# prakharg24/yoloret

Hardware: AMD Instinct MI355X
Metric: images/sec (+ p50 per-image ms) MobileNetV2-0.75x @416, 1/2/4/8 MI355X (higher is better)
Workload: dtype f32; 1 GPU; mobilenetv2x75 @416, batch 64 per GPU, fp32, random weights (SURVEY 8(d) recipe; parity tests run the variance-preserving recipe, see DESIGN.md 5), C=20: forward + decode + per-class NMS + pack; 3 steps in flight (each step = one whole batch on its own HIP stream and workspace); global_batch=64, parallelism=dp1 (image-sharded)

## Files before the change

### yoloret_amd/csrc/pointwise_stream.hip

```cpp
#include <algorithm>
#include <cstdlib>

#include "pws_common.h"
#include "mbr_common.h"

typedef __attribute__((address_space(3))) void* pwt_lds_ptr;

struct PwtDiv { unsigned m; int s; };
static inline PwtDiv pwt_div_make(unsigned d) {
    if (d <= 1) return {0u, -1};
    int l = 0;
    while ((1u << l) < d) ++l;
    const unsigned long long m = ((1ull << (31 + l)) + d - 1) / d;
    return {(unsigned)m, l - 1};
}
__device__ __forceinline__ int pwt_div(int n, PwtDiv d) { return d.s < 0 ? n : (int)(__umulhi((unsigned)n, d.m) >> d.s); }

struct PwtArgs {
    const float* planes;
    unsigned plane_bytes;
    int T;
    int csplit;
    int nwg;
    int ntiles;
    PwtDiv d_hw, d_wq, d_hwq;
    unsigned in_bytes, out_bytes, gate_bytes;
    int TA, quad;
    unsigned out2_bytes;
};

#ifndef PWT_MAX_WAVES
#define PWT_MAX_WAVES 16
#endif
constexpr int pwt_waves_fit(int nk, int rows, int mode);
constexpr int pwt_waves(int nk, int rows, int mode) { return pwt_waves_fit(nk, rows, mode) < PWT_MAX_WAVES ? pwt_waves_fit(nk, rows, mode) : PWT_MAX_WAVES; }
constexpr int pwt_waves_fit(int nk, int rows, int mode) {
    const int nkr = nk * rows;
    if (mode == 0) return nkr <= 6 ? 16 : nkr <= 10 ? 12 : 8;
    if (mode == 1) return nkr <= 9 ? 16 : nkr <= 12 ? 12 : 8;
    if (rows == 1) return nk <= 8 ? 16 : nk <= 10 ? 12 : 8;
    return nk <= 2 ? 16 : nk <= 4 ? 12 : 8;
}

#ifdef PWT_TIMING
__device__ unsigned pwt_dbg[256 * 16 * 8];
extern "C" int yr_pwt_dbg_read(unsigned* dst, int n) { return (int)hipMemcpyFromSymbol(dst, HIP_SYMBOL(pwt_dbg), (size_t)n * 4); }
#define PWT_T(i) { __builtin_amdgcn_sched_barrier(0); const unsigned long long t_ = __builtin_amdgcn_s_memtime(); tacc[i] += t_ - tlast; tlast = t_; __builtin_amdgcn_sched_barrier(0); }
#else
#define PWT_T(i)
#endif

__device__ __forceinline__ int pwt_pixel_of_row(const PwArgs& a, const PwtArgs& x, int m) {
    if (!x.quad) return m;
    const int q = m >> 2, sub = m & 3;
    const int wq = a.W >> 1, hwq = (a.H >> 1) * wq;
    const int b = pwt_div(q, x.d_hwq), r = q - b * hwq;
    const int yq = pwt_div(r, x.d_wq), xq = r - yq * wq;
    return (b * a.H + 2 * yq + (sub >> 1)) * a.W + 2 * xq + (sub & 1);
}

template <int NK, int ROWS, int MODE>
__global__ __launch_bounds__(64 * pwt_waves(NK, ROWS, MODE)) void pwt_kernel(PwArgs a, PwtArgs x) {
    constexpr int NW = pwt_waves(NK, ROWS, MODE), TB = NK * 2048;
    typedef unsigned u4 __attribute__((ext_vector_type(4)));
    extern __shared__ __attribute__((aligned(16))) char lds_raw[];
    const int lane = threadIdx.x & 63, li = lane & 15, g = lane >> 4;
    const int w = __builtin_amdgcn_readfirstlane(threadIdx.x >> 6);
    const int part = blockIdx.x % x.csplit, wg = blockIdx.x / x.csplit;
    const int t0 = part * x.T / x.csplit, t1 = (part + 1) * x.T / x.csplit, run = t1 - t0;
    float* const ss = reinterpret_cast<float*>(lds_raw + (size_t)run * TB);
#ifdef PWT_TIMING
    unsigned long long tacc[8] = {0, 0, 0, 0, 0, 0, 0, 0}, tlast = __builtin_amdgcn_s_memtime();
#endif

    {
        const yr_rsrc wsrc = yr_make_rsrc(x.planes, x.plane_bytes);
        const int npiece = run * NK * 2;
        for (int p = w; p < npiece; p += NW)
            __builtin_amdgcn_raw_ptr_buffer_load_lds(wsrc, (pwt_lds_ptr)(lds_raw + p * 1024), 16, (unsigned)(t0 * TB + p * 1024 + lane * 16), 0, 0, 0);
    }
    const int bn_i = (int)threadIdx.x;
    const int bn_n = bn_i < 16 * run && (a.out2 != nullptr || 16 * t0 + bn_i < a.N) ? 16 * t0 + bn_i : 0;
    const float bn_sl = (a.scale ? a.scale : x.planes)[bn_n], bn_hl = (a.shift ? a.shift : x.planes)[bn_n];

    const int kp = a.S.kp;
    const int stride = x.nwg * NW;
    int tile = wg + x.nwg * w;
    const yr_rsrc xsrc = yr_make_rsrc(a.S.s[0].ptr, x.in_bytes), osrc = yr_make_rsrc(a.out, x.out_bytes);
    const yr_rsrc osrc2 = yr_make_rsrc(a.out2 ? a.out2 : a.out, a.out2 ? x.out2_bytes : 16u);
    const yr_rsrc gsrc = yr_make_rsrc(MODE == 2 ? a.gate : a.S.s[0].ptr, MODE == 2 ? x.gate_bytes : 16u);
    PwRow<0> row[MODE == 0 ? ROWS : 1];
    float4 xa[ROWS][NK][2];
    int cv[MODE == 0 ? ROWS : 1][MODE == 0 ? NK : 1][2];
    unsigned goff[ROWS];
    int pix[ROWS];
    constexpr int GQ = 2, NGQ = (NK + GQ - 1) / GQ;
    float4 gq[MODE == 2 ? 2 : 1][MODE == 2 ? ROWS : 1][GQ][2];
    auto gate_issue = [&](auto J) __attribute__((always_inline)) {
        constexpr int j = decltype(J)::value;
        if constexpr (MODE == 2 && j < NGQ) {
            pw_unroll<ROWS * GQ * 2>([&](auto U) __attribute__((always_inline)) {
                constexpr int u = decltype(U)::value, i = u / (2 * GQ), cc = (u / 2) % GQ, q = u % 2, c = j * GQ + cc;
                const int k = c * 32 + g * 8 + 4 * q;
                if constexpr (c < NK) gq[j & 1][i][cc][q] = __builtin_bit_cast(float4, __builtin_amdgcn_raw_buffer_load_b128(gsrc, k < kp ? goff[i] + 4u * k : YR_DEAD, 0, 0));
            });
        }
    };
    const int csrc = a.S.s[0].c, ldsrc = a.S.s[0].ld;
    auto fetch = [&]() __attribute__((always_inline)) {
#pragma unroll
        for (int i = 0; i < ROWS; ++i) {
            const int m = (tile * ROWS + i) * 16 + li;
            if constexpr (MODE == 0) {
                row[i].init(a, m);
                pix[i] = pw_pixel_of_row(a, m < a.M ? m : 0);
                pw_unroll<NK * 2>([&](auto U) __attribute__((always_inline)) {
                    constexpr int u = decltype(U)::value, c = u / 2, q = u % 2;
                    float4 unused;
                    row[i].template issue<false>(a, c * 32 + g * 8 + 4 * q, kp, xa[i][c][q], unused, cv[i][c][q]);
                });
            } else {
                const int mm = pwt_pixel_of_row(a, x, m < a.M ? m : 0);
                pix[i] = mm;
                const unsigned poff = (unsigned)mm * (unsigned)ldsrc * 4u;
                if constexpr (MODE == 2) goff[i] = (unsigned)pwt_div(mm, x.d_hw) * (unsigned)a.gate_ld * 4u;
                pw_unroll<NK * 2>([&](auto U) __attribute__((always_inline)) {
                    constexpr int u = decltype(U)::value, c = u / 2, q = u % 2;
                    const int k = c * 32 + g * 8 + 4 * q;
                    xa[i][c][q] = __builtin_bit_cast(float4, __builtin_amdgcn_raw_buffer_load_b128(xsrc, (m < a.M && k < kp) ? poff + 4u * k : YR_DEAD, 0, 0));
                });
            }
        }
        gate_issue(std::integral_constant<int, 0>{});
    };
    auto no_fetch = [&]() __attribute__((always_inline)) {
        pw_unroll<ROWS * NK * 2>([&](auto U) __attribute__((always_inline)) {
            constexpr int u = decltype(U)::value;
            xa[u / (2 * NK)][(u / 2) % NK][u % 2] = make_float4(0.f, 0.f, 0.f, 0.f);
            if constexpr (MODE == 0) cv[u / (2 * NK)][(u / 2) % NK][u % 2] = 0;
        });
    };
    if (tile < x.ntiles) fetch();
    else no_fetch();
    PWT_T(0)
    if (bn_i < 16 * run) { ss[bn_i] = a.scale ? bn_sl : 1.f; ss[16 * run + bn_i] = a.shift ? bn_hl : 0.f; }
    __builtin_amdgcn_s_waitcnt(0x0070);
    __syncthreads();
    PWT_T(1)

    const f32x4 k11 = {0.00048828125f, 0.00048828125f, 0.00048828125f, 0.00048828125f};
    const bool ragged = (csrc & 3) != 0, clamp = a.act != YR_ACT_NONE;
    while (tile < x.ntiles) {
        pws_u4 xh[ROWS][NK], xm[ROWS][NK];
        pw_unroll<ROWS * NK>([&](auto U) __attribute__((always_inline)) {
            constexpr int u = decltype(U)::value, c = u / ROWS, i = u % ROWS;
            float4 v0 = xa[i][c][0], v1 = xa[i][c][1];
            if constexpr (MODE == 0) {
                v0 = pw_finish<1>(v0, v0, cv[i][c][0]);
                v1 = pw_finish<1>(v1, v1, cv[i][c][1]);
            } else {
                const int k0 = c * 32 + g * 8;
                if constexpr (MODE == 2) {
                    if constexpr (i == 0 && c % GQ == 0) gate_issue(std::integral_constant<int, c / GQ + 1>{});
                    const float4 g0 = gq[(c / GQ) & 1][i][c % GQ][0], g1 = gq[(c / GQ) & 1][i][c % GQ][1];
                    v0 = make_float4(v0.x * g0.x, v0.y * g0.y, v0.z * g0.z, v0.w * g0.w);
                    v1 = make_float4(v1.x * g1.x, v1.y * g1.y, v1.z * g1.z, v1.w * g1.w);
                }
                if (ragged) {
                    v0 = pw_finish<1>(v0, v0, csrc - k0);
                    v1 = pw_finish<1>(v1, v1, csrc - k0 - 4);
                }
            }
            unsigned h[4], mm[4];
            yr_cut2(v0.x, v0.y, h[0], mm[0]);
            yr_cut2(v0.z, v0.w, h[1], mm[1]);
            yr_cut2(v1.x, v1.y, h[2], mm[2]);
            yr_cut2(v1.z, v1.w, h[3], mm[3]);
            xh[i][c] = (pws_u4){h[0], h[1], h[2], h[3]};
            xm[i][c] = (pws_u4){mm[0], mm[1], mm[2], mm[3]};
        });
        PWT_T(2)
        unsigned obase[ROWS], obase2[ROWS];
#pragma unroll
        for (int i = 0; i < ROWS; ++i) {
            const int m = (tile * ROWS + i) * 16 + li;
            const bool keep = m < a.M && (!a.pool || (li & 3) == 0), keep2 = m < a.M && (!a.pool2 || (li & 3) == 0);
            obase[i] = keep ? (unsigned)(a.pool ? m >> 2 : pix[i]) * (unsigned)a.out_ld * 4u : YR_DEAD;
            obase2[i] = keep2 && a.out2 ? (unsigned)(a.pool2 ? m >> 2 : pix[i]) * (unsigned)a.out2_ld * 4u : YR_DEAD;
        }
        for (int t = 0; t < run; ++t) {
            const pws_u4* fe = reinterpret_cast<const pws_u4*>(lds_raw + (size_t)t * TB) + lane;
            f32x4 acc[ROWS], ac1[ROWS];
#pragma unroll
            for (int i = 0; i < ROWS; ++i) { acc[i] = (f32x4){0.f, 0.f, 0.f, 0.f}; ac1[i] = acc[i]; }
#pragma unroll
            for (int c = 0; c < NK; ++c) {
                const pws_u4 wh = fe[(2 * c) * 64], wm = fe[(2 * c + 1) * 64];
#pragma unroll
                for (int i = 0; i < ROWS; ++i) acc[i] = pws_mfma(wh, xh[i][c], acc[i]);
#pragma unroll
                for (int i = 0; i < ROWS; ++i) ac1[i] = pws_mfma(wh, xm[i][c], ac1[i]);
#pragma unroll
                for (int i = 0; i < ROWS; ++i) ac1[i] = pws_mfma(wm, xh[i][c], ac1[i]);
            }
            const f32x4 sc = *reinterpret_cast<const f32x4*>(ss + 16 * t + 4 * g);
            const f32x4 sh = *reinterpret_cast<const f32x4*>(ss + 16 * run + 16 * t + 4 * g);
            const bool second = t0 + t >= x.TA;
            const int n = 16 * (t0 + t - (second ? x.TA : 0)) + 4 * g, cnt = (second ? a.N2 : a.N) - n;
            const bool clamp_t = second ? a.act2 != YR_ACT_NONE : clamp, pool_t = second ? a.pool2 != 0 : a.pool != 0;
#pragma unroll
            for (int i = 0; i < ROWS; ++i) {
                f32x4 v = __builtin_elementwise_fma(ac1[i], k11, acc[i]);
#pragma unroll
                for (int r = 0; r < 4; ++r) v[r] = __builtin_fmaf(v[r], sc[r], sh[r]);
                if (clamp_t) {
#pragma unroll
                    for (int r = 0; r < 4; ++r) v[r] = __builtin_amdgcn_fmed3f(v[r], 0.f, 6.f);
                }
                if (pool_t) {
#pragma unroll
                    for (int r = 0; r < 4; ++r) {
                        v[r] = fmaxf(v[r], __int_as_float(__builtin_amdgcn_update_dpp(0, __float_as_int(v[r]), 0xB1, 0xf, 0xf, false)));
                        v[r] = fmaxf(v[r], __int_as_float(__builtin_amdgcn_update_dpp(0, __float_as_int(v[r]), 0x4E, 0xf, 0xf, false)));
                    }
                }
                const unsigned ob = second ? obase2[i] : obase[i];
                const unsigned off = ob == YR_DEAD || cnt <= 0 ? YR_DEAD : ob + 4u * (unsigned)n;
                if (second) {
                    if (cnt >= 4) __builtin_amdgcn_raw_buffer_store_b128(__builtin_bit_cast(u4, v), osrc2, off, 0, 0);
                    else {
#pragma unroll
                        for (int r = 0; r < 3; ++r) __builtin_amdgcn_raw_buffer_store_b32(__float_as_uint(v[r]), osrc2, r < cnt ? off + 4u * r : YR_DEAD, 0, 0);
                    }
                } else if (cnt >= 4) {
                    __builtin_amdgcn_raw_buffer_store_b128(__builtin_bit_cast(u4, v), osrc, off, 0, 0);
                } else {
#pragma unroll
                    for (int r = 0; r < 3; ++r) __builtin_amdgcn_raw_buffer_store_b32(__float_as_uint(v[r]), osrc, r < cnt ? off + 4u * r : YR_DEAD, 0, 0);
                }
            }
        }
        PWT_T(3)
        tile += stride;
        if (tile < x.ntiles) fetch();
        else no_fetch();
        PWT_T(4)
#ifdef PWT_TIMING
        tacc[5] += 1;
#endif
    }
#ifdef PWT_TIMING
    __builtin_amdgcn_s_waitcnt(0x0070);
    PWT_T(6)
    if (lane < 8 && blockIdx.x < 256) {
        unsigned tv = 0;
#pragma unroll
        for (int i = 0; i < 8; ++i) tv = lane == i ? (unsigned)tacc[i] : tv;
        pwt_dbg[(blockIdx.x * 16 + w) * 8 + lane] = tv;
    }
#endif
}

template <int NK, int ROWS>
static int launch_pwt(const PwArgs& a, PwtArgs& x, hipStream_t s) {
    const int mode = pw_mode_of(a);
    const int NW = pwt_waves(NK, ROWS, mode);
    x.ntiles = (a.M + 16 * ROWS - 1) / (16 * ROWS);
    int cs = 1;
    while ((x.T + cs - 1) / cs * (size_t)(NK * 2048 + 128) > 150 * 1024 && cs < x.T) ++cs;
    x.csplit = cs;
    const int cus = 256 / cs;
    int aw = (x.ntiles + cus - 1) / cus;
    if (aw > NW) aw = NW;
    x.nwg = (x.ntiles + aw - 1) / aw;
    if (x.nwg > cus) x.nwg = cus;
    const size_t lds = (size_t)((x.T + cs - 1) / cs) * (NK * 2048 + 128);
    YR_REQUIRE(lds <= 160 * 1024 && (x.T + cs - 1) / cs <= 32, "pointwise (pixel-stationary form): %d tiles of %d chunks do not fit LDS", x.T, NK);
    const dim3 grid((unsigned)(x.nwg * cs));
#define PWT_GO(MD) YR_LAUNCH((pwt_kernel<NK, ROWS, MD>), grid, dim3(64 * pwt_waves(NK, ROWS, MD)), lds, 160 * 1024, s, ("pwt_kernel<%d,%d,%d>", NK, ROWS, MD), a, x)
    return mode == 0 ? PWT_GO(0) : mode == 1 ? PWT_GO(1) : PWT_GO(2);
#undef PWT_GO
}

extern "C" int yr_pwt_chunks(int kp) {
    static const int sizes[] = {1, 2, 3, 4, 5, 6, 7, 8, 9, 10, 12, 16};
    const int nk = (kp + 31) / 32;
    for (int v : sizes)
        if (v >= nk) return v;
    return 0;
}

static int pwt_launch_images(const PwArgs& a, hipStream_t s) {
    const int nk = yr_pwt_chunks(a.S.kp);
    YR_REQUIRE(nk > 0, "pointwise (pixel-stationary form): a k space of %d channels is beyond 16 chunks", a.S.kp);
    YR_REQUIRE(a.dw_w == nullptr && a.pre == nullptr && a.res == nullptr, "pointwise (pixel-stationary form): no depthwise-folded source, addend or residual");
    YR_REQUIRE(a.act == YR_ACT_NONE || a.act == YR_ACT_RELU6, "pointwise (pixel-stationary form): activation %d (none and ReLU6 only)", a.act);
    YR_REQUIRE(!pw_any_pooled(a.S), "pointwise (pixel-stationary form): no pooled source");
    PwtArgs x;
    x.TA = (a.N + 15) / 16;
    x.planes = a.wt; x.T = x.TA + (a.out2 ? (a.N2 + 15) / 16 : 0);
    x.quad = a.pool || (a.out2 && a.pool2);
    if (a.out2) YR_REQUIRE(pw_mode_of(a) != 0, "pointwise (pixel-stationary form): two outputs need a single identity source");
    if (a.out2) YR_REQUIRE(a.act2 == YR_ACT_NONE || a.act2 == YR_ACT_RELU6, "pointwise (pixel-stationary form): activation %d of the second output", a.act2);
    if (x.quad) YR_REQUIRE(a.H % 2 == 0 && a.W % 2 == 0, "pointwise (pixel-stationary form): a pooled output needs an even map");
    x.plane_bytes = (unsigned)x.T * (unsigned)nk * 2048u;
    x.d_hw = pwt_div_make((unsigned)(a.H * a.W));
    x.d_wq = pwt_div_make((unsigned)(a.W >> 1 > 0 ? a.W >> 1 : 1));
    x.d_hwq = pwt_div_make((unsigned)((a.H >> 1) * (a.W >> 1) > 0 ? (a.H >> 1) * (a.W >> 1) : 1));
    const long long inb = (long long)a.M * a.S.s[0].ld * 4, outb = (long long)(a.pool ? a.M / 4 : a.M) * a.out_ld * 4;
    YR_REQUIRE(inb < (long long)YR_DEAD && outb < (long long)YR_DEAD, "pointwise (pixel-stationary form): a map of %lld bytes is beyond the 32-bit offsets", inb > outb ? inb : outb);
    x.in_bytes = (unsigned)inb; x.out_bytes = (unsigned)outb;
    const long long outb2 = a.out2 ? (long long)(a.pool2 ? a.M / 4 : a.M) * a.out2_ld * 4 : 0;
    YR_REQUIRE(outb2 < (long long)YR_DEAD, "pointwise (pixel-stationary form): a second output of %lld bytes is beyond the 32-bit offsets", outb2);
    x.out2_bytes = (unsigned)outb2;
    x.gate_bytes = a.gate ? (unsigned)((long long)(a.M / (a.H * a.W)) * a.gate_ld * 4) : 0u;
    const char* rows_env = getenv("YR_PWT_ROWS");
    const bool two = rows_env && atoi(rows_env) == 2 && nk <= 6;
#define PWT_CASE(K) if (nk == K) return two ? launch_pwt<K, 2>(a, x, s) : launch_pwt<K, 1>(a, x, s);
#define PWT_CASE1(K) if (nk == K) return launch_pwt<K, 1>(a, x, s);
#ifdef PWT_ONLY
    PWT_CASE(PWT_ONLY)
#else
    PWT_CASE(1) PWT_CASE(2) PWT_CASE(3) PWT_CASE(4) PWT_CASE(5) PWT_CASE(6) PWT_CASE1(7) PWT_CASE1(8) PWT_CASE1(9) PWT_CASE1(10) PWT_CASE1(12) PWT_CASE1(16)
#endif
#undef PWT_CASE
#undef PWT_CASE1
    return YR_ERR_ARG;
}

int yr_pw_launch_stream(const PwArgs& a0, hipStream_t s) {
    const long long hw = (long long)a0.H * a0.W;
    const int B = (int)(a0.M / hw);
    long long per_image = (a0.pool ? hw / 4 : hw) * a0.out_ld * 4;
    if (a0.out2) per_image = std::max(per_image, (a0.pool2 ? hw / 4 : hw) * a0.out2_ld * 4);
    for (int i = 0; i < a0.S.n; ++i) per_image = std::max(per_image, (long long)a0.S.s[i].h * a0.S.s[i].w * a0.S.s[i].ld * 4);
    const char* lim = getenv("YR_PWT_MAX_BYTES");
    const long long fit = (lim && atoll(lim) > 0 ? atoll(lim) : 0x7e000000ll) / (per_image > 0 ? per_image : 1);
    if (fit >= B || (long long)B * hw != a0.M) return pwt_launch_images(a0, s);
    YR_REQUIRE(fit >= 1, "pointwise (pixel-stationary form): one image's map of %lld bytes is beyond the 32-bit offsets", per_image);
    for (int b0 = 0; b0 < B; b0 += (int)fit) {
        PwArgs a = a0;
        const int n = B - b0 < fit ? B - b0 : (int)fit;
        a.M = (int)(n * hw);
        for (int i = 0; i < a.S.n; ++i) a.S.s[i].ptr += (size_t)b0 * a.S.s[i].h * a.S.s[i].w * a.S.s[i].ld;
        if (a.gate) a.gate += (size_t)b0 * a.gate_ld;
        a.out += (size_t)b0 * (a.pool ? hw / 4 : hw) * a.out_ld;
        if (a.out2) a.out2 += (size_t)b0 * (a.pool2 ? hw / 4 : hw) * a.out2_ld;
        const int rc = pwt_launch_images(a, s);
        if (rc) return rc;
    }
    return YR_OK;
}
```

Baseline: 50960 img/s.

## Rework pixel-stationary pointwise geometry: wider channel split, runtime wave count, async BN loads

Launch geometry now comes from a helper that splits output-channel tiles across more workgroups (about one part per six tiles, capped by available wave slots). When the split leaves slack it drops to 8 waves per workgroup, and the workgroup count accounts for several workgroups sharing a CU's LDS. Wave count becomes a runtime parameter, and an env override is added for tuning. BN scale/shift are now loaded straight into LDS with buffer-to-LDS loads instead of through registers. The start-up wait only drains the weight and BN loads rather than the in-flight pixel fetches, using s_barrier instead of __syncthreads. The 16-wave threshold for rows==1 gate mode is also lowered. The wider split means more redundant activation reads, and the partial vmcnt wait relies on exact load-ordering counts.

```diff
diff --git a/yoloret_amd/csrc/pointwise_stream.hip b/yoloret_amd/csrc/pointwise_stream.hip
--- a/yoloret_amd/csrc/pointwise_stream.hip
+++ b/yoloret_amd/csrc/pointwise_stream.hip
@@ -1,5 +1,6 @@
 #include <algorithm>
 #include <cstdlib>
+#include <cstring>
 
 #include "pws_common.h"
 #include "mbr_common.h"
@@ -22,6 +23,7 @@
     int T;
     int csplit;
     int nwg;
+    int nw;
     int ntiles;
     PwtDiv d_hw, d_wq, d_hwq;
     unsigned in_bytes, out_bytes, gate_bytes;
@@ -38,7 +40,7 @@
     const int nkr = nk * rows;
     if (mode == 0) return nkr <= 6 ? 16 : nkr <= 10 ? 12 : 8;
     if (mode == 1) return nkr <= 9 ? 16 : nkr <= 12 ? 12 : 8;
-    if (rows == 1) return nk <= 8 ? 16 : nk <= 10 ? 12 : 8;
+    if (rows == 1) return nk <= 7 ? 16 : nk <= 10 ? 12 : 8;
     return nk <= 2 ? 16 : nk <= 4 ? 12 : 8;
 }
 
@@ -61,7 +63,7 @@
 
 template <int NK, int ROWS, int MODE>
 __global__ __launch_bounds__(64 * pwt_waves(NK, ROWS, MODE)) void pwt_kernel(PwArgs a, PwtArgs x) {
-    constexpr int NW = pwt_waves(NK, ROWS, MODE), TB = NK * 2048;
+    constexpr int TB = NK * 2048;
     typedef unsigned u4 __attribute__((ext_vector_type(4)));
     extern __shared__ __attribute__((aligned(16))) char lds_raw[];
     const int lane = threadIdx.x & 63, li = lane & 15, g = lane >> 4;
@@ -69,6 +71,7 @@
     const int part = blockIdx.x % x.csplit, wg = blockIdx.x / x.csplit;
     const int t0 = part * x.T / x.csplit, t1 = (part + 1) * x.T / x.csplit, run = t1 - t0;
     float* const ss = reinterpret_cast<float*>(lds_raw + (size_t)run * TB);
+    const int ru = (16 * run + 63) & ~63;
 #ifdef PWT_TIMING
     unsigned long long tacc[8] = {0, 0, 0, 0, 0, 0, 0, 0}, tlast = __builtin_amdgcn_s_memtime();
 #endif
@@ -76,15 +79,22 @@
     {
         const yr_rsrc wsrc = yr_make_rsrc(x.planes, x.plane_bytes);
         const int npiece = run * NK * 2;
-        for (int p = w; p < npiece; p += NW)
+        for (int p = w; p < npiece; p += x.nw)
             __builtin_amdgcn_raw_ptr_buffer_load_lds(wsrc, (pwt_lds_ptr)(lds_raw + p * 1024), 16, (unsigned)(t0 * TB + p * 1024 + lane * 16), 0, 0, 0);
-    }
-    const int bn_i = (int)threadIdx.x;
-    const int bn_n = bn_i < 16 * run && (a.out2 != nullptr || 16 * t0 + bn_i < a.N) ? 16 * t0 + bn_i : 0;
-    const float bn_sl = (a.scale ? a.scale : x.planes)[bn_n], bn_hl = (a.shift ? a.shift : x.planes)[bn_n];
+        const unsigned bn_bytes = (unsigned)(a.out2 ? 16 * x.T : a.N) * 4u;
+        const yr_rsrc csrc_ = yr_make_rsrc(a.scale ? a.scale : x.planes, a.scale ? bn_bytes : 0u);
+        const yr_rsrc hsrc_ = yr_make_rsrc(a.shift ? a.shift : x.planes, a.shift ? bn_bytes : 0u);
+        for (int i = 64 * w; i < 16 * run; i += 64 * x.nw) {
+            const unsigned off = (unsigned)(16 * t0 + i + lane) * 4u;
+            if (a.scale) __builtin_amdgcn_raw_ptr_buffer_load_lds(csrc_, (pwt_lds_ptr)(ss + i), 4, off, 0, 0, 0);
+            else ss[i + lane] = 1.f;
+            if (a.shift) __builtin_amdgcn_raw_ptr_buffer_load_lds(hsrc_, (pwt_lds_ptr)(ss + ru + i), 4, off, 0, 0, 0);
+            else ss[ru + i + lane] = 0.f;
+        }
+    }
 
     const int kp = a.S.kp;
-    const int stride = x.nwg * NW;
+    const int stride = x.nwg * x.nw;
     int tile = wg + x.nwg * w;
     const yr_rsrc xsrc = yr_make_rsrc(a.S.s[0].ptr, x.in_bytes), osrc = yr_make_rsrc(a.out, x.out_bytes);
     const yr_rsrc osrc2 = yr_make_rsrc(a.out2 ? a.out2 : a.out, a.out2 ? x.out2_bytes : 16u);
@@ -140,12 +150,19 @@
             if constexpr (MODE == 0) cv[u / (2 * NK)][(u / 2) % NK][u % 2] = 0;
         });
     };
-    if (tile < x.ntiles) fetch();
-    else no_fetch();
-    PWT_T(0)
-    if (bn_i < 16 * run) { ss[bn_i] = a.scale ? bn_sl : 1.f; ss[16 * run + bn_i] = a.shift ? bn_hl : 0.f; }
-    __builtin_amdgcn_s_waitcnt(0x0070);
-    __syncthreads();
+    constexpr int NPIX = MODE == 0 ? 0 : ROWS * NK * 2;
+    static_assert(NPIX < 64, "vmcnt is a 6-bit count");
+    if (tile < x.ntiles) {
+        fetch();
+        PWT_T(0)
+        __builtin_amdgcn_sched_barrier(0);
+        __builtin_amdgcn_s_waitcnt(0x0070 | (NPIX & 15) | ((NPIX >> 4) << 14));
+    } else {
+        no_fetch();
+        PWT_T(0)
+        __builtin_amdgcn_s_waitcnt(0x0070);
+    }
+    __builtin_amdgcn_s_barrier();
     PWT_T(1)
 
     const f32x4 k11 = {0.00048828125f, 0.00048828125f, 0.00048828125f, 0.00048828125f};
@@ -204,7 +221,7 @@
                 for (int i = 0; i < ROWS; ++i) ac1[i] = pws_mfma(wm, xh[i][c], ac1[i]);
             }
             const f32x4 sc = *reinterpret_cast<const f32x4*>(ss + 16 * t + 4 * g);
-            const f32x4 sh = *reinterpret_cast<const f32x4*>(ss + 16 * run + 16 * t + 4 * g);
+            const f32x4 sh = *reinterpret_cast<const f32x4*>(ss + ru + 16 * t + 4 * g);
             const bool second = t0 + t >= x.TA;
             const int n = 16 * (t0 + t - (second ? x.TA : 0)) + 4 * g, cnt = (second ? a.N2 : a.N) - n;
             const bool clamp_t = second ? a.act2 != YR_ACT_NONE : clamp, pool_t = second ? a.pool2 != 0 : a.pool != 0;
@@ -261,23 +278,61 @@
 #endif
 }
 
+struct PwtGeometry { int cs, nw, nwg; };
+constexpr int PWT_CUS = 256;
+static inline size_t pwt_lds_bytes(int T, int nk, int cs) {
+    const int run = (T + cs - 1) / cs;
+    return (size_t)run * (size_t)(nk * 2048) + 8u * (size_t)((16 * run + 63) & ~63);
+}
+static inline int pwt_nwg(int T, int nk, int nw_max, int ntiles, int cs, int nw) {
+    const int by_lds = (int)((size_t)(160 * 1024) / pwt_lds_bytes(T, nk, cs));
+    int per_cu = nw_max / nw < by_lds ? nw_max / nw : by_lds;
+    if (per_cu < 1) per_cu = 1;
+    int cap = PWT_CUS * per_cu / cs;
+    if (cap < 1) cap = 1;
+    int aw = (ntiles + cap - 1) / cap;
+    if (aw > nw) aw = nw;
+    const int nwg = (ntiles + aw - 1) / aw;
+    return nwg < cap ? nwg : cap;
+}
+static inline PwtGeometry pwt_geometry(int T, int nk, int nw_max, int ntiles) {
+    PwtGeometry g;
+    g.cs = 1;
+    while ((size_t)((T + g.cs - 1) / g.cs) * (size_t)(nk * 2048 + 128) > 150 * 1024 && g.cs < T) ++g.cs;
+    g.nw = nw_max;
+    const int slots = PWT_CUS * nw_max;
+    int want = (T + 2) / 6;
+    if (want > slots / (ntiles > 0 ? ntiles : 1)) want = slots / (ntiles > 0 ? ntiles : 1);
+    if (want > g.cs) g.cs = want;
+    if (ntiles * g.cs <= slots && g.cs > 1 && nw_max > 8) g.nw = 8;
+    g.nwg = pwt_nwg(T, nk, nw_max, ntiles, g.cs, g.nw);
+    return g;
+}
+
 template <int NK, int ROWS>
 static int launch_pwt(const PwArgs& a, PwtArgs& x, hipStream_t s) {
     const int mode = pw_mode_of(a);
     const int NW = pwt_waves(NK, ROWS, mode);
     x.ntiles = (a.M + 16 * ROWS - 1) / (16 * ROWS);
-    int cs = 1;
-    while ((x.T + cs - 1) / cs * (size_t)(NK * 2048 + 128) > 150 * 1024 && cs < x.T) ++cs;
-    x.csplit = cs;
-    const int cus = 256 / cs;
-    int aw = (x.ntiles + cus - 1) / cus;
-    if (aw > NW) aw = NW;
-    x.nwg = (x.ntiles + aw - 1) / aw;
-    if (x.nwg > cus) x.nwg = cus;
-    const size_t lds = (size_t)((x.T + cs - 1) / cs) * (NK * 2048 + 128);
-    YR_REQUIRE(lds <= 160 * 1024 && (x.T + cs - 1) / cs <= 32, "pointwise (pixel-stationary form): %d tiles of %d chunks do not fit LDS", x.T, NK);
+    PwtGeometry g = pwt_geometry(x.T, NK, NW, x.ntiles);
+    if (const char* env = getenv("YR_PWT_GEOMETRY")) {
+        int v[3] = {0, 0, 0};
+        for (int i = 0; i < 3 && env && *env; ++i) {
+            v[i] = atoi(env);
+            env = strchr(env, ',');
+            if (env) ++env;
+        }
+        YR_REQUIRE(v[0] >= 0 && v[1] >= 0 && v[2] >= 0 && v[2] <= 65536, "pointwise (pixel-stationary form): YR_PWT_GEOMETRY=%d,%d,%d", v[0], v[1], v[2]);
+        if (v[0]) g.cs = v[0] < x.T ? v[0] : x.T;
+        if (v[1]) g.nw = v[1] < NW ? v[1] : NW;
+        g.nwg = v[2] ? v[2] : pwt_nwg(x.T, NK, NW, x.ntiles, g.cs, g.nw);
+    }
+    const int cs = g.cs;
+    x.csplit = cs; x.nw = g.nw; x.nwg = g.nwg;
+    const size_t lds = pwt_lds_bytes(x.T, NK, cs);
+    YR_REQUIRE(lds <= 160 * 1024, "pointwise (pixel-stationary form): %d tiles of %d chunks in %d parts do not fit LDS", x.T, NK, cs);
     const dim3 grid((unsigned)(x.nwg * cs));
-#define PWT_GO(MD) YR_LAUNCH((pwt_kernel<NK, ROWS, MD>), grid, dim3(64 * pwt_waves(NK, ROWS, MD)), lds, 160 * 1024, s, ("pwt_kernel<%d,%d,%d>", NK, ROWS, MD), a, x)
+#define PWT_GO(MD) YR_LAUNCH((pwt_kernel<NK, ROWS, MD>), grid, dim3(64 * x.nw), lds, 160 * 1024, s, ("pwt_kernel<%d,%d,%d>", NK, ROWS, MD), a, x)
     return mode == 0 ? PWT_GO(0) : mode == 1 ? PWT_GO(1) : PWT_GO(2);
 #undef PWT_GO
 }
```

Measured after the change: 51130 img/s (median of 6 runs). No clear change (+0.3%).
